# leggedrobotics/art_planner

Hardware: AMD Instinct MI355X
Metric: validated states/sec on 400x400@0.04m map (sample + validity check) (higher is better)
Workload: dtype f32; 1 GPU; C2: lazy_prm_star_min_update front end, 400x400@0.04m Perlin terrain (seed 1234) + 12 obstacles, YAML robot, batch sampler + validity checker; map=400x400@0.04, lanes=1

## Files before the change

### art_planner_amd/csrc/artp_capi.hip

```cpp
#include "../../include/artp_c.h"

#include <hip/hip_runtime.h>
#include <hipcub/hipcub.hpp>

#include <cmath>
#include <cstdio>
#include <atomic>
#include <chrono>
#include <cstdlib>
#include <cstring>
#include <mutex>
#include <string>
#include <array>
#include <vector>

#include "device_scratch.h"
#include "pinned_buffer.h"
#include "pipeline.h"
#include "cost_kernels.h"

using namespace artp;

#define ARTP_FEW_STATES 16
#define ARTP_SVC_MAX_STATES 2
// ... 1236 lines not shown
  if (exit_codes) HIP_TRY(c, hipMemcpyAsync(exit_codes, d_ec, n, hipMemcpyDeviceToHost, c->lane->stream));
  return check_error_flag(c);
}

int artp_validate_states_dev(artp_ctx* c, const double* se3, size_t n, uint8_t* valid, int8_t* detail) {
  if (!c || (n && (!se3 || !valid))) return ARTP_ERR_INVALID_ARG;
  std::lock_guard<std::recursive_mutex> lock(c->mu);
  if (!c->have_field[0] || !c->have_field[1]) return ARTP_ERR_NO_MAP;
  if (n == 0) return ARTP_OK;
  HIP_TRY(c, hipSetDevice(c->device));
  if (!detail && n <= ARTP_FEW_STATES) {
    hipLaunchKernelGGL(validate_few_kernel, dim3((unsigned)n), dim3(320), lds_few(c), c->lane->stream, c->field[0],
                       c->field[1], c->geom, c->robot, se3, n, valid, c->caps_full, c->caps_foot_full, c->lane->d_error.get(), 0u);
    HIP_TRY(c, hipGetLastError());
    return ARTP_OK;
  }
  if (detail) {
    hipLaunchKernelGGL(validate_states_kernel<1>, dim3(grid_full(c, n)), dim3(64), lds_full(c), c->lane->stream,
                       c->field[0], c->field[1], c->geom, c->robot, se3, n, valid, detail, c->caps_full,
                       c->lane->d_error.get(), (unsigned long long*)nullptr);
    HIP_TRY(c, hipGetLastError());
    return ARTP_OK;
  }
  return launch_validate_pipeline(c, se3, n, valid);
}

int artp_validate_states(artp_ctx* c, const double* se3, size_t n, uint8_t* valid, int8_t* detail) {
  if (!c || (n && (!se3 || !valid))) return ARTP_ERR_INVALID_ARG;
  if (n == 0) return ARTP_OK;
  std::lock_guard<std::recursive_mutex> lock(c->mu);
  HIP_TRY(c, hipSetDevice(c->device));
  if (!detail && n <= ARTP_FEW_STATES) {
    if (!c->have_field[0] || !c->have_field[1]) return ARTP_ERR_NO_MAP;
    if (c->svc_enabled && n <= ARTP_SVC_MAX_STATES) return svc_validate(c, se3, n, valid);
    std::memcpy(c->pin_states.host(), se3, n * 7 * sizeof(double));
    for (size_t i = 0; i < n; ++i) c->pin_labels.host()[i] = 0;
    const unsigned tag = 0x80u;
    hipLaunchKernelGGL(validate_few_kernel, dim3((unsigned)n), dim3(320), lds_few(c), c->lane->stream, c->field[0],
                       c->field[1], c->geom, c->robot, (const double*)c->pin_states.dev(), n,
                       (volatile uint8_t*)c->pin_labels.dev(), c->caps_full, c->caps_foot_full, c->lane->d_error.get(), tag);
    HIP_TRY(c, hipGetLastError());
    bool done = false;
    if (c->poll_labels) {
      const auto t0 = std::chrono::steady_clock::now();
      for (unsigned spin = 0; !done; ++spin) {
        done = true;
        for (size_t i = 0; i < n; ++i) done = done && (c->pin_labels.host()[i] & 0x80u);
        if (!done && (spin & 1023u) == 1023u &&
            std::chrono::steady_clock::now() - t0 > std::chrono::milliseconds(2))
          break;
      }
    }
    if (!done) HIP_TRY(c, hipStreamSynchronize(c->lane->stream));
    bool overflow = false;
    for (size_t i = 0; i < n; ++i) {
      valid[i] = c->pin_labels.host()[i] & 1u;
      overflow = overflow || (c->pin_labels.host()[i] & 2u);
    }
    if (overflow) {
      c->last_error = "a box window exceeded the LDS tile capacity";
      return ARTP_ERR_CAPACITY;
    }
    return ARTP_OK;
  }
  ARTP_TRY(ensure_scratch(c, c->lane->host_args, n * 7 * sizeof(double)));
  ARTP_TRY(ensure_scratch(c, c->lane->host_results, n * 7));
  HIP_TRY(c, hipMemcpyAsync(c->lane->host_args.get(), se3, n * 7 * sizeof(double), hipMemcpyHostToDevice, c->lane->stream));
  uint8_t* d_valid = c->lane->host_results.as<uint8_t>();
  int8_t* d_detail = reinterpret_cast<int8_t*>(d_valid + n);
  ARTP_TRY(artp_validate_states_dev(c, c->lane->host_args.as<const double>(), n, d_valid,
                                detail ? d_detail : nullptr));
  HIP_TRY(c, hipMemcpyAsync(valid, d_valid, n, hipMemcpyDeviceToHost, c->lane->stream));
  if (detail) HIP_TRY(c, hipMemcpyAsync(detail, d_detail, n * 6, hipMemcpyDeviceToHost, c->lane->stream));
  return check_error_flag(c);
}

static int pack_sampler_tables(artp_ctx* c, int rows, int cols);

static int ensure_sampler_storage(artp_ctx* c, int rows, int cols) {
  if (c->sampler_buf.get() && c->sampler_pack.get() && c->sampler_rows == rows && c->sampler_cols == cols) return ARTP_OK;
  const size_t e = (size_t)rows * cols;
  const int npiv = (cols + 15) / 16, pitch = npiv * 16, ppitch = (npiv + 3) & ~3;
  const size_t floats = (size_t)rows * pitch + (size_t)rows * ppitch + 8 * e + 64;
  for (lane_state& l : c->lanes)
    if (&l != c->lane && l.init) HIP_TRY(c, hipStreamSynchronize(l.stream));
  HIP_TRY(c, hipStreamSynchronize(c->lane->stream));
  c->have_sampler = false;
  c->sampler_rows = c->sampler_cols = 0;
  HIP_TRY(c, c->sampler_buf.reset());
  HIP_TRY(c, c->sampler_pack.reset());
  HIP_TRY(c, c->sampler_buf.reserve((6 * e + rows) * sizeof(float)));
  HIP_TRY(c, c->sampler_pack.reserve(floats * sizeof(float)));
  c->sampler_rows = rows;
  c->sampler_cols = cols;
  return ARTP_OK;
}

int artp_upload_sampler_layers(artp_ctx* c, const float* cum_prob, const float* cum_prob_rowwise,
                               const float* elevation, const float* normal_x, const float* normal_y,
                               const float* normal_z, const float* plane_fit_std_dev, int rows,
                               int cols, double len_x, double len_y, double pos_x, double pos_y) {
  if (!c || !cum_prob || !cum_prob_rowwise || !elevation || !normal_x || !normal_y || !normal_z ||
      !plane_fit_std_dev || rows < 1 || cols < 1)
    return ARTP_ERR_INVALID_ARG;
  std::lock_guard<std::recursive_mutex> lock(c->mu);
  HIP_TRY(c, hipSetDevice(c->device));
  const size_t e = (size_t)rows * cols;
  c->map_version.fetch_add(1, std::memory_order_release);
  ARTP_TRY(ensure_sampler_storage(c, rows, cols));
  ARTP_TRY(order_after_other_lanes(c));
  float* p = c->sampler_buf.get();
  const float* src[6] = {cum_prob, elevation, normal_x, normal_y, normal_z, plane_fit_std_dev};
  const float** dst[6] = {&c->sampler.cum_prob, &c->sampler.elevation, &c->sampler.normal_x,
                          &c->sampler.normal_y, &c->sampler.normal_z, &c->sampler.plane_fit_std_dev};
  for (int k = 0; k < 6; ++k) {
    HIP_TRY(c, hipMemcpyAsync(p, src[k], e * sizeof(float), hipMemcpyHostToDevice, c->lane->stream));
    *dst[k] = p;
    p += e;
  }
  HIP_TRY(c, hipMemcpyAsync(p, cum_prob_rowwise, rows * sizeof(float), hipMemcpyHostToDevice, c->lane->stream));
  c->sampler.cum_prob_rowwise = p;
  HIP_TRY(c, hipStreamSynchronize(c->lane->stream));
  ARTP_TRY(pack_sampler_tables(c, rows, cols));
  if (!c->have_geom) {
    c->geom.len_x = len_x; c->geom.len_y = len_y; c->geom.pos_x = pos_x; c->geom.pos_y = pos_y;
    c->geom.rows = rows; c->geom.cols = cols; c->geom.res = len_x / rows;
    c->have_geom = true;
  }
  c->sampler.from_distribution = c->params.sample_from_distribution;
  c->have_sampler = true;
  return publish_map_write(c);
}

static int pack_sampler_tables(artp_ctx* c, int rows, int cols) {
  const size_t e = (size_t)rows * cols;
  const int npiv = (cols + 15) / 16, pitch = npiv * 16, ppitch = (npiv + 3) & ~3;
  const size_t floats = (size_t)rows * pitch + (size_t)rows * ppitch + 8 * e + 64;
  HIP_TRY(c, hipMemsetAsync(c->sampler_pack.get(), 0, floats * sizeof(float), c->lane->stream));
  float* cells = c->sampler_pack.get();
  float* cdf_t = cells + 8 * e;
  float* piv = cdf_t + (size_t)rows * pitch;
  c->sampler.npiv = npiv;
  c->sampler.pitch = pitch;
  c->sampler.ppitch = ppitch;
  hipLaunchKernelGGL(sampler_pack_kernel, dim3((unsigned)((e + 255) / 256)), dim3(256), 0, c->lane->stream, c->sampler, rows,
                     cols, cdf_t, piv, reinterpret_cast<float4*>(cells));
  HIP_TRY(c, hipGetLastError());
  c->sampler.cells = reinterpret_cast<const float4*>(cells);
  c->sampler.cum_prob_t = cdf_t;
  c->sampler.pivots = piv;
  HIP_TRY(c, hipStreamSynchronize(c->lane->stream));
  return ARTP_OK;
}

static int upload_sampler_layers_from_device(artp_ctx* c, const float* cum_prob, const float* cum_prob_rowwise,
                                      const float* elevation, const float* normal_x, const float* normal_y,
                                      const float* normal_z, const float* plane_fit_std_dev, int rows, int cols,
                                      double len_x, double len_y, double pos_x, double pos_y) {
  std::lock_guard<std::recursive_mutex> lock(c->mu);
  HIP_TRY(c, hipSetDevice(c->device));
  const size_t e = (size_t)rows * cols;
  c->map_version.fetch_add(1, std::memory_order_release);
  ARTP_TRY(ensure_sampler_storage(c, rows, cols));
  ARTP_TRY(order_after_other_lanes(c));
  float* p = c->sampler_buf.get();
  const float* src[6] = {cum_prob, elevation, normal_x, normal_y, normal_z, plane_fit_std_dev};
  const float** dst[6] = {&c->sampler.cum_prob, &c->sampler.elevation, &c->sampler.normal_x,
                          &c->sampler.normal_y, &c->sampler.normal_z, &c->sampler.plane_fit_std_dev};
  for (int k = 0; k < 6; ++k) {
    HIP_TRY(c, hipMemcpyAsync(p, src[k], e * sizeof(float), hipMemcpyDeviceToDevice, c->lane->stream));
    *dst[k] = p;
    p += e;
  }
  HIP_TRY(c, hipMemcpyAsync(p, cum_prob_rowwise, rows * sizeof(float), hipMemcpyDeviceToDevice, c->lane->stream));
  c->sampler.cum_prob_rowwise = p;
  HIP_TRY(c, hipStreamSynchronize(c->lane->stream));
  ARTP_TRY(pack_sampler_tables(c, rows, cols));
  if (!c->have_geom) {
    c->geom.len_x = len_x; c->geom.len_y = len_y; c->geom.pos_x = pos_x; c->geom.pos_y = pos_y;
    c->geom.rows = rows; c->geom.cols = cols; c->geom.res = len_x / rows;
    c->have_geom = true;
  }
  c->sampler.from_distribution = c->params.sample_from_distribution;
  c->have_sampler = true;
  return publish_map_write(c);
}

static int finite_min_max_dev(artp_ctx* c, const float* d_layer, size_t n, float* lo, float* hi, bool* any) {
  std::lock_guard<std::recursive_mutex> lock(c->mu);
  HIP_TRY(c, hipSetDevice(c->device));
  int init[2] = {0x7fffffff, (int)0x80000000};
  int* d_keys = reinterpret_cast<int*>(c->lane->d_count.get());
  HIP_TRY(c, hipMemcpyAsync(d_keys, init, sizeof(init), hipMemcpyHostToDevice, c->lane->stream));
  hipLaunchKernelGGL(finite_min_max_kernel, dim3((unsigned)std::min<size_t>((n + 255) / 256, (size_t)c->n_cus)), dim3(256), 0,
                     c->lane->stream, d_layer, (int)n, d_keys);
  HIP_TRY(c, hipGetLastError());
  int keys[2];
  HIP_TRY(c, hipMemcpyAsync(keys, d_keys, sizeof(keys), hipMemcpyDeviceToHost, c->lane->stream));
  HIP_TRY(c, hipStreamSynchronize(c->lane->stream));
  *any = keys[0] <= keys[1];
  auto unkey = [](int k) {
    const int i = k >= 0 ? k : k ^ 0x7fffffff;
    float v;
    std::memcpy(&v, &i, 4);
    return v;
  };
  *lo = unkey(keys[0]);
  *hi = unkey(keys[1]);
  return ARTP_OK;
}

static int launch_sampler(artp_ctx* c, uint64_t seed, uint64_t first_index, size_t n, double* se3_out, PoseRec* recs) {
  const size_t blocks = (n + 255) / 256;
  if (blocks > 0x7fffffffull) {
    c->last_error = "batch too large for one sampler launch";
    return ARTP_ERR_INVALID_ARG;
  }
  if (c->sampler.from_distribution)
    hipLaunchKernelGGL(sample_states_kernel<true>, dim3((unsigned)blocks), dim3(256), 0, c->lane->stream, c->sampler,
                       c->geom, c->robot, seed, first_index, n, se3_out, c->field[0], recs);
  else
    hipLaunchKernelGGL(sample_states_kernel<false>, dim3((unsigned)blocks), dim3(256), 0, c->lane->stream, c->sampler,
                       c->geom, c->robot, seed, first_index, n, se3_out, c->field[0], recs);
  HIP_TRY(c, hipGetLastError());
  return ARTP_OK;
}

int artp_sample_states_dev(artp_ctx* c, uint64_t seed, uint64_t first_index, size_t n, double* se3_out) {
  if (!c || (n && !se3_out)) return ARTP_ERR_INVALID_ARG;
  std::lock_guard<std::recursive_mutex> lock(c->mu);
  if (!c->have_sampler) return ARTP_ERR_NO_MAP;
  if (n == 0) return ARTP_OK;
  HIP_TRY(c, hipSetDevice(c->device));
  return launch_sampler(c, seed, first_index, n, se3_out, nullptr);
}

int artp_sample_states(artp_ctx* c, uint64_t seed, uint64_t first_index, size_t n, double* se3_out) {
  if (!c || (n && !se3_out)) return ARTP_ERR_INVALID_ARG;
  if (n == 0) return ARTP_OK;
  std::lock_guard<std::recursive_mutex> lock(c->mu);
  HIP_TRY(c, hipSetDevice(c->device));
  ARTP_TRY(ensure_scratch(c, c->lane->host_args, n * 7 * sizeof(double)));
  ARTP_TRY(artp_sample_states_dev(c, seed, first_index, n, c->lane->host_args.as<double>()));
  HIP_TRY(c, hipMemcpyAsync(se3_out, c->lane->host_args.get(), n * 7 * sizeof(double), hipMemcpyDeviceToHost, c->lane->stream));
  HIP_TRY(c, hipStreamSynchronize(c->lane->stream));
  return ARTP_OK;
}

int artp_sample_and_validate_dev(artp_ctx* c, uint64_t seed, uint64_t first_index, size_t n,
                                 double* se3_out, uint8_t* valid_out, size_t* n_valid) {
  if (!c || (n && (!se3_out || !valid_out))) return ARTP_ERR_INVALID_ARG;
  std::lock_guard<std::recursive_mutex> lock(c->mu);
  if (!c->have_sampler || !c->have_field[0] || !c->have_field[1]) return ARTP_ERR_NO_MAP;
  if (n == 0) {
    if (n_valid) *n_valid = 0;
    return ARTP_OK;
  }
  if (n >= (1ull << 32)) {
    c->last_error = "batch too large (state index is 32 bit)";
    return ARTP_ERR_INVALID_ARG;
  }
  HIP_TRY(c, hipSetDevice(c->device));
  ARTP_TRY(ensure_recs(c, n));
  if (n <= ARTP_FEW_STATES) {
    ARTP_TRY(launch_sampler(c, seed, first_index, n, se3_out, nullptr));
    ARTP_TRY(artp_validate_states_dev(c, se3_out, n, valid_out, nullptr));
  } else {
    ARTP_TRY(launch_sampler(c, seed, first_index, n, se3_out, c->lane->pose_recs.as<PoseRec>()));
  }
  if (n > ARTP_FEW_STATES) {
    ARTP_TRY(launch_validate_pipeline(c, se3_out, n, valid_out, true));
  }
  if (n_valid) {
    HIP_TRY(c, hipMemsetAsync(c->lane->d_count.get(), 0, sizeof(unsigned long long), c->lane->stream));
    size_t blocks = (n / 16 + 255) / 256 + 1;
    if (blocks > (size_t)c->n_cus * 4) blocks = (size_t)c->n_cus * 4;
    hipLaunchKernelGGL(count_valid_kernel, dim3((unsigned)blocks), dim3(256), 0, c->lane->stream,
                       (const uint8_t*)valid_out, n, c->lane->d_count.get());
    HIP_TRY(c, hipGetLastError());
  }
  if (n_valid) {
    unsigned long long cnt = 0;
    HIP_TRY(c, hipMemcpyAsync(&cnt, c->lane->d_count.get(), sizeof(cnt), hipMemcpyDeviceToHost, c->lane->stream));
    HIP_TRY(c, hipStreamSynchronize(c->lane->stream));
    *n_valid = (size_t)cnt;
  }
  return ARTP_OK;
}

int artp_sample_and_validate(artp_ctx* c, uint64_t seed, uint64_t first_index, size_t n, double* se3_out,
                             uint8_t* valid_out, uint64_t* map_version) {
  if (!c || (n && (!se3_out || !valid_out))) return ARTP_ERR_INVALID_ARG;
  std::lock_guard<std::recursive_mutex> lock(c->mu);
  if (map_version) *map_version = c->map_version.load(std::memory_order_acquire);
  if (n == 0) return ARTP_OK;
  HIP_TRY(c, hipSetDevice(c->device));
  ARTP_TRY(ensure_scratch(c, c->lane->host_args, n * 7 * sizeof(double)));
  ARTP_TRY(ensure_scratch(c, c->lane->host_results, n));
  ARTP_TRY(artp_sample_and_validate_dev(c, seed, first_index, n, c->lane->host_args.as<double>(),
                                    c->lane->host_results.as<uint8_t>(), nullptr));
  HIP_TRY(c, hipMemcpyAsync(se3_out, c->lane->host_args.get(), n * 7 * sizeof(double), hipMemcpyDeviceToHost, c->lane->stream));
  HIP_TRY(c, hipMemcpyAsync(valid_out, c->lane->host_results.get(), n, hipMemcpyDeviceToHost, c->lane->stream));
  return check_error_flag(c);
}

int artp_set_r3_extent(artp_ctx* c, double max_extent) {
// ... 1701 lines not shown
```

### art_planner_amd/csrc/artp_math.h

```cpp
#pragma once

#include <hip/hip_runtime.h>
#include <stdint.h>

#define ARTP_HD __host__ __device__ __forceinline__
#define ARTP_EPS 1.1920928955078125e-07f

namespace artp {

struct FieldDev {
  const float* data;
  int nW, nD;
  float width, depth, half_w, half_d;
  float sample_w, sample_d, inv_w, inv_d, zx_aspect;
  float pos[3];
  float R[12];
  int has_nan;
  float partner_tol;
  const unsigned char* partner_flags;
  int partner_R;
};

template <class T>
ARTP_HD T gather32(const T* __restrict__ base, unsigned idx) {
  return *reinterpret_cast<const T*>(reinterpret_cast<const char*>(base) + idx * (unsigned)sizeof(T));
}

struct BoxHF {
  float pos[3];
  float R[9];
  float side[3];
  float aabb[6];
  int minX, maxX, minZ, maxZ;
  int on_field;
};

ARTP_HD float dot3(float a0, float a1, float a2, float b0, float b1, float b2) {
  return a0 * b0 + a1 * b1 + a2 * b2;
}

ARTP_HD bool is_finite(float v) { return (__float_as_uint(v) & 0x7f800000u) != 0x7f800000u; }
ARTP_HD bool is_nan(float v) { return v != v; }

ARTP_HD float next_toward_neg_inf(float x) {
  uint32_t u = __float_as_uint(x);
  if ((u & 0x7f800000u) == 0x7f800000u) return x;
  if ((u << 1) == 0u) return __uint_as_float(0x80000001u);
  return __uint_as_float((u & 0x80000000u) ? u + 1u : u - 1u);
}
ARTP_HD float next_toward_pos_inf(float x) {
  uint32_t u = __float_as_uint(x);
  if ((u & 0x7f800000u) == 0x7f800000u) return x;
  if ((u << 1) == 0u) return __uint_as_float(0x00000001u);
  return __uint_as_float((u & 0x80000000u) ? u - 1u : u + 1u);
}

ARTP_HD void safe_normalize3(float& a0, float& a1, float& a2) {
  const float abs0 = fabsf(a0), abs1 = fabsf(a1), abs2 = fabsf(a2);
  int idx;
  if (abs1 > abs0) {
    idx = (abs2 > abs1) ? 2 : 1;
  } else if (abs2 > abs0) {
    idx = 2;
  } else {
    if (!(abs0 > 0.0f)) return;
    idx = 0;
  }
  const float big = idx == 0 ? a0 : (idx == 1 ? a1 : a2);
  const float first = idx == 0 ? a1 : a0;
  const float second = idx == 2 ? a1 : a2;
  const float recip = 1.0f / fabsf(big);
  const float p1 = first * recip, p2 = second * recip;
  const float l = 1.0f / sqrtf(1.0f + p1 * p1 + p2 * p2);
  const float nb = copysignf(l, big), n1 = p1 * l, n2 = p2 * l;
  a0 = idx == 0 ? nb : n1;
  a1 = idx == 1 ? nb : (idx == 0 ? n1 : n2);
  a2 = idx == 2 ? nb : n2;
}

ARTP_HD void orthogonalize_R9(float& m0, float& m1, float& m2, float& m4, float& m5, float& m6, float& m8,
                              float& m9, float& m10) {
  if (!(m0 != 0.0f || m1 != 0.0f || m2 != 0.0f)) return;
  const float n0 = m0 * m0 + m1 * m1 + m2 * m2;
  const float proj = dot3(m0, m1, m2, m4, m5, m6);
  float r0 = m4, r1 = m5, r2 = m6;
  const bool in_place = !(proj != 0);
  if (!in_place) {
    const float pd = proj / n0;
    r0 = m4 - pd * m0;
    r1 = m5 - pd * m1;
    r2 = m6 - pd * m2;
  }
  if (!(r0 != 0.0f || r1 != 0.0f || r2 != 0.0f)) return;
  if (n0 != 1.0f) safe_normalize3(m0, m1, m2);
  const float n1 = r0 * r0 + r1 * r1 + r2 * r2;
  if (n1 != 1.0f) safe_normalize3(r0, r1, r2);
  if (in_place) {
    m4 = r0;
    m5 = r1;
    m6 = r2;
  }
  m8 = m1 * r2 - m2 * r1;
  m9 = m2 * r0 - m0 * r2;
  m10 = m0 * r1 - m1 * r0;
}

ARTP_HD void orthogonalize_R(float* m) {
  orthogonalize_R9(m[0], m[1], m[2], m[4], m[5], m[6], m[8], m[9], m[10]);
// ... 253 lines not shown
```

### art_planner_amd/csrc/kernels.h

```cpp
#pragma once

#include "box_check.h"

namespace artp {

struct RobotDev {
  float torso[3];
  float foot[3];
  float torso_off[3];
  float feet_off_x, feet_off_y;
  int unknown_space_untraversable;
  double reach_z;
  double max_pitch_pert, max_roll_pert;
};

struct MapGeom {
  double len_x, len_y, pos_x, pos_y, res;
  int rows, cols;
};

struct SamplerDev {
  int from_distribution;
  const float* cum_prob;
  const float* cum_prob_rowwise;
// ... 54 lines not shown
  return s;
}

__device__ __forceinline__ bool map_is_inside(const MapGeom& g, double px, double py) {
  const double tx = -((px - g.pos_x) - 0.5 * g.len_x);
  const double ty = -((py - g.pos_y) - 0.5 * g.len_y);
  return tx >= 0.0 && ty >= 0.0 && tx < g.len_x && ty < g.len_y;
}

template <int WAVES>
__global__ void __launch_bounds__(64 * WAVES)
check_boxes_kernel(FieldDev f, float sx, float sy, float sz, const float* __restrict__ poses,
                   size_t n, uint8_t* __restrict__ hit, uint8_t* __restrict__ exit_codes,
                   ScratchCaps caps, int* __restrict__ error_flag) {
  extern __shared__ __attribute__((aligned(16))) char smem[];
  const int lane = threadIdx.x & 63;
  const int wave_in_block = threadIdx.x >> 6;
  const WaveScratch s = carve_scratch(smem, wave_in_block, caps);
  const size_t wave0 = (size_t)blockIdx.x * WAVES + wave_in_block;
  const size_t stride = (size_t)gridDim.x * WAVES;
  for (size_t i = wave0; i < n; i += stride) {
    float pose[16];
#pragma unroll
    for (int k = 0; k < 16; ++k) pose[k] = poses[16 * i + k];
    BoxHF b;
    setup_box(f, pose, sx, sy, sz, b);
    int ec;
    const int r = wave_check_box(f, b, s, lane, &ec);
    if (r < 0) {
      if (lane == 0) atomicExch(error_flag, 1);
    }
    if (lane == 0) {
      hit[i] = (uint8_t)(r > 0);
      if (exit_codes) exit_codes[i] = (uint8_t)(ec < 0 ? 255 : ec);
    }
    wave_lds_sync();
  }
}

__device__ __forceinline__ void rot_from_quat(float x, float y, float z, float w, float R[9]) {
  const float tx = 2.0f * x, ty = 2.0f * y, tz = 2.0f * z;
  const float twx = tx * w, twy = ty * w, twz = tz * w;
  const float txx = tx * x, txy = ty * x, txz = tz * x;
  const float tyy = ty * y, tyz = tz * y, tzz = tz * z;
  R[0] = 1.0f - (tyy + tzz);
  R[1] = txy - twz;
  R[2] = txz + twy;
  R[3] = txy + twz;
  R[4] = 1.0f - (txx + tzz);
  R[5] = tyz - twx;
  R[6] = txz - twy;
  R[7] = tyz + twx;
  R[8] = 1.0f - (txx + tyy);
}

__device__ __forceinline__ void pose3_from_se3(const double* se3, float t[3], float R[9]) {
  t[0] = (float)se3[0];
  t[1] = (float)se3[1];
  t[2] = (float)se3[2];
  rot_from_quat((float)se3[3], (float)se3[4], (float)se3[5], (float)se3[6], R);
}

struct __attribute__((aligned(16))) PoseRec {
  float t[3];
  float q[4];
  float bR[9];
};

__device__ __forceinline__ void make_pose_rec(const FieldDev& f, const double* se3, float4 out[4]) {
  float t[3], R[9], bR[9];
  pose3_from_se3(se3, t, R);
  box_rotation_in_field(f, R, bR);
  out[0] = make_float4(t[0], t[1], t[2], (float)se3[3]);
  out[1] = make_float4((float)se3[4], (float)se3[5], (float)se3[6], bR[0]);
  out[2] = make_float4(bR[1], bR[2], bR[3], bR[4]);
  out[3] = make_float4(bR[5], bR[6], bR[7], bR[8]);
}

__device__ __forceinline__ int rec_stage_slot(int l, int k) { return 4 * l + ((k + (l >> 2)) & 3); }
__device__ __forceinline__ void stage_pose_rec(float4* rw, int lane, const float4 r[4]) {
#pragma unroll
  for (int k = 0; k < 4; ++k) rw[rec_stage_slot(lane, k)] = r[k];
}
__device__ __forceinline__ void flush_pose_recs(const float4* rw, int lane, size_t live, PoseRec* __restrict__ dst_recs) {
  float4* dst = reinterpret_cast<float4*>(dst_recs);
#pragma unroll
  for (int k = 0; k < 4; ++k) {
    const int j = k * 64 + lane;
    typedef float native_f4 __attribute__((ext_vector_type(4)));
    if ((size_t)j < live * 4)
      __builtin_nontemporal_store(reinterpret_cast<const native_f4*>(rw)[rec_stage_slot(j >> 2, j & 3)],
                                  reinterpret_cast<native_f4*>(dst) + j);
  }
}

__global__ void __launch_bounds__(256)
pose_rec_kernel(FieldDev f, const double* __restrict__ se3, size_t n, PoseRec* __restrict__ recs) {
  __shared__ double stage[4][64 * 8];
  const int lane = threadIdx.x & 63;
  double* sw = stage[threadIdx.x >> 6];
  const size_t i0 = (size_t)blockIdx.x * blockDim.x + (threadIdx.x - lane);
  if (i0 >= n) return;
  const size_t live = n - i0 < 64 ? n - i0 : 64;
  const double* in = se3 + 7 * i0;
  double v7[7];
#pragma unroll
  for (int k = 0; k < 7; ++k) v7[k] = in[(size_t)(k * 64 + lane) < live * 7 ? k * 64 + lane : 0];
#pragma unroll
  for (int k = 0; k < 7; ++k)
    if ((size_t)(k * 64 + lane) < live * 7) sw[k * 64 + lane] = v7[k];
  wave_lds_sync();
  float4 r[4];
  const bool have = (size_t)lane < live;
  if (have) {
    double st[7];
#pragma unroll
    for (int j = 0; j < 7; ++j) st[j] = sw[lane * 7 + j];
    make_pose_rec(f, st, r);
  }
  wave_lds_sync();
  float4* rw = reinterpret_cast<float4*>(sw);
  if (have) stage_pose_rec(rw, lane, r);
  wave_lds_sync();
  flush_pose_recs(rw, lane, live, recs + i0);
}

__device__ __forceinline__ int wave_state_valid(const FieldDev& fb, const FieldDev& ff,
                                                const MapGeom& g, const RobotDev& rb,
                                                const double* se3, const WaveScratch& s, int lane,
                                                int8_t* detail6) {
  float t[3], R[9];
  pose3_from_se3(se3, t, R);
  if (detail6 && lane == 0) {
#pragma unroll
    for (int k = 0; k < 5; ++k) detail6[k] = -2;
    detail6[5] = 0;
  }
  int valid = 1;
  int err = 0;
  for (int k = 0; k < 5 && valid; ++k) {
    const bool body = (k == 0);
    const float ox = body ? rb.torso_off[0] : ((k <= 2) ? rb.feet_off_x : -rb.feet_off_x);
    const float oy = body ? rb.torso_off[1] : ((k & 1) ? rb.feet_off_y : -rb.feet_off_y);
    const float oz = body ? rb.torso_off[2] : 0.0f;
    float pose[16];
    pose[0] = (R[0] * ox + (R[1] * oy + R[2] * oz)) + t[0];
    pose[1] = (R[3] * ox + (R[4] * oy + R[5] * oz)) + t[1];
    pose[2] = (R[6] * ox + (R[7] * oy + R[8] * oz)) + t[2];
    pose[3] = 0.0f;
#pragma unroll
    for (int r = 0; r < 3; ++r) {
      pose[4 + 4 * r + 0] = R[3 * r + 0];
      pose[4 + 4 * r + 1] = R[3 * r + 1];
      pose[4 + 4 * r + 2] = R[3 * r + 2];
      pose[4 + 4 * r + 3] = 0.0f;
    }
    const bool inside = map_is_inside(g, (double)pose[0], (double)pose[1]);
    int ok;
    int ec = -1;
    if (!inside) {
      ok = body ? 1 : !rb.unknown_space_untraversable;
    } else {
      const FieldDev& fk = body ? fb : ff;
      BoxHF b;
      setup_box(fk, pose, body ? rb.torso[0] : rb.foot[0], body ? rb.torso[1] : rb.foot[1],
                body ? rb.torso[2] : rb.foot[2], b);
      int r = wave_check_box(fk, b, s, lane, &ec);
      wave_lds_sync();
      if (r < 0) {
        err = 1;
        r = 0;
      }
      ok = body ? !r : r;
// ... 134 lines not shown
  unsigned long long t_idle = t_start;
  uint32_t served = 0;
  const volatile uint32_t* line = reinterpret_cast<const volatile uint32_t*>(mb);
  for (;;) {
    if (k == 0) {
      uint32_t leave = 0, w = 0, seq;
      for (;;) {
        if (lane < 16) w = line[lane];
        seq = (uint32_t)__builtin_amdgcn_readfirstlane((int)w);
        if (seq != last_seq) break;
        const uint32_t nq = (uint32_t)__builtin_amdgcn_readlane((int)w, 1);
        const unsigned long long now = wall_clock64();
        if ((nq & 0x100u) || now - t_idle > ARTP_SVC_IDLE_TICKS || now - t_start > ARTP_SVC_LIFE_TICKS) {
          leave = 1;
          break;
        }
        __builtin_amdgcn_s_sleep(4);
      }
      if (!leave && lane < 16) w = line[lane];
      if (lane < 16) s_line[lane] = w;
      if (!leave && ((uint32_t)__builtin_amdgcn_readlane((int)w, 1) & 0xffu) > 1u && lane < 14)
        s_line[16 + lane] = reinterpret_cast<const volatile uint32_t*>(mb->state1)[lane];
      if (lane == 0) s_exit = leave;
    }
    __syncthreads();
    if (s_exit) {
      if (threadIdx.x == 0) {
        mb->running = 0u;
        __threadfence_system();
      }
      return;
    }
    const uint32_t seq = s_line[0];
    uint32_t n = s_line[1] & 0xffu;
    n = n < 1u ? 1u : (n > 2u ? 2u : n);
    uint32_t bits = 0;
    for (uint32_t i = 0; i < n; ++i) {
      double st[7];
#pragma unroll
      for (int j = 0; j < 7; ++j) {
        const uint32_t lo = s_line[(i ? 16 : 2) + 2 * j], hi = s_line[(i ? 16 : 2) + 2 * j + 1];
        st[j] = __longlong_as_double((long long)(((unsigned long long)hi << 32) | lo));
      }
      const int ok = few_box_ok(fb, ff, g, rb, st, k, s, lane);
      wave_lds_sync();
      if (lane == 0) box_ok[k] = ok;
      __syncthreads();
      if (threadIdx.x == 0) {
        bool err = false, v = true;
#pragma unroll
        for (int q = 0; q < 5; ++q) {
          err = err || box_ok[q] < 0;
          v = v && box_ok[q] > 0;
        }
        bits |= ((v && !err ? 1u : 0u) | (err ? 2u : 0u)) << (2 * i);
      }
      __syncthreads();
    }
    if (threadIdx.x == 0) {
      mb->resp = (seq << 8) | bits;
      __threadfence_system();
      ++served;
      mb->served = served;
    }
    last_seq = seq;
    t_idle = wall_clock64();
    __syncthreads();
  }
}

ARTP_HD double uniform01(uint64_t seed, uint64_t index, unsigned k) {
  uint64_t x = seed + 0x9E3779B97F4A7C15ULL * (index * 8u + (uint64_t)k + 1u);
  x ^= x >> 30;
  x *= 0xBF58476D1CE4E5B9ULL;
  x ^= x >> 27;
  x *= 0x94D049BB133111EBULL;
  x ^= x >> 31;
  x += seed;
  x ^= x >> 30;
  x *= 0xBF58476D1CE4E5B9ULL;
  x ^= x >> 27;
  x *= 0x94D049BB133111EBULL;
  x ^= x >> 31;
  return (double)(x >> 11) * (1.0 / 9007199254740992.0);
}

__device__ __forceinline__ void sincos_half_angle(double x, double* sn, double* cs) {
  const double kf = rint(x * 6.36619772367581382433e-01);
  const int k = (int)kf;
  double r = fma(-kf, 1.57079632673412561417e+00, x);
  r = fma(-kf, 6.07710050650619224932e-11, r);
  const double z = r * r;
  const double ps = fma(z, fma(z, fma(z, fma(z, fma(z, 1.58969099521155010221e-10, -2.50507602534068634195e-08),
                                                 2.75573137070700676789e-06),
                                          -1.98412698298579493134e-04),
                                   8.33333333332248946124e-03),
                        -1.66666666666666324348e-01);
  const double pc = fma(z, fma(z, fma(z, fma(z, fma(z, -1.13596475577881948265e-11, 2.08757232129817482790e-09),
                                                 -2.75573143513906633035e-07),
                                          2.48015872894767294178e-05),
                                   -1.38888888888741095749e-03),
                        4.16666666666666019037e-02);
  const double s0 = fma(r * z, ps, r);
  const double c0 = fma(z * z, pc, fma(-0.5, z, 1.0));
  const bool swap = (k & 1) != 0;
  const double sa = swap ? c0 : s0, ca = swap ? s0 : c0;
  *sn = (k & 2) ? -sa : sa;
  *cs = ((k + 1) & 2) ? -ca : ca;
}

template <bool FROM_DIST>
__device__ __forceinline__ void sample_one(const SamplerDev& sm, const MapGeom& g, const RobotDev& rb,
                                           uint64_t seed, uint64_t index, double out[7], const float* row_cdf) {
  double px, py;
  int cell_row = 0, cell_col = 0;
  if (FROM_DIST) {
    const double samp_col = uniform01(seed, index, 0);
    const double samp_row = uniform01(seed, index, 1);
    int lo = 0, hi = g.rows - 1;
    while (lo < hi) {
      const int mid = (lo + hi) >> 1;
      if ((double)row_cdf[mid] > samp_row) hi = mid; else lo = mid + 1;
    }
    const int row = lo;
    const float* prow = sm.pivots + (size_t)row * sm.ppitch;
    const int nch = sm.ppitch >> 2;
    if (nch <= 8) {
      const float uf = __double2float_rd(samp_col);
      const float4* p4 = reinterpret_cast<const float4*>(prow);
      lo = 0;
#pragma unroll
      for (int h = 0; h < 2; ++h) {
        float4 pv[4];
#pragma unroll
        for (int k = 0; k < 4; ++k)
          if (4 * h + k < nch) pv[k] = p4[4 * h + k];
#pragma unroll
        for (int k = 0; k < 4; ++k)
          if (4 * h + k < nch)
            lo += (!(pv[k].x > uf) ? 1 : 0) + (!(pv[k].y > uf) ? 1 : 0) + (!(pv[k].z > uf) ? 1 : 0) +
                  (!(pv[k].w > uf) ? 1 : 0);
      }
    } else {
      lo = 0;
      hi = sm.npiv - 1;
      while (lo < hi) {
        const int mid = (lo + hi) >> 1;
        if ((double)prow[mid] > samp_col) hi = mid; else lo = mid + 1;
      }
    }
    const int c0 = lo << 4;
    const int c1 = (c0 + 15 < g.cols - 1) ? c0 + 15 : g.cols - 1;
    const float4* grp = reinterpret_cast<const float4*>(sm.cum_prob_t + (size_t)row * sm.pitch + c0);
    int below = 0;
    const float uf_col = __double2float_rd(samp_col);
#pragma unroll
    for (int q4 = 0; q4 < 4; ++q4) {
      const float4 v = grp[q4];
      below += (c0 + 4 * q4 + 0 <= c1 && !(v.x > uf_col)) ? 1 : 0;
      below += (c0 + 4 * q4 + 1 <= c1 && !(v.y > uf_col)) ? 1 : 0;
      below += (c0 + 4 * q4 + 2 <= c1 && !(v.z > uf_col)) ? 1 : 0;
      below += (c0 + 4 * q4 + 3 <= c1 && !(v.w > uf_col)) ? 1 : 0;
    }
    const int col = (c0 + below < c1) ? c0 + below : c1;
    cell_row = row;
    cell_col = col;
    px = (g.pos_x + (0.5 * g.len_x - 0.5 * g.res)) + g.res * (double)(-row);
    py = (g.pos_y + (0.5 * g.len_y - 0.5 * g.res)) + g.res * (double)(-col);
  } else {
    const double lx = g.pos_x - g.len_x, hx = g.pos_x + g.len_x;
    const double ly = g.pos_y - g.len_y, hy = g.pos_y + g.len_y;
    for (unsigned a = 0;; ++a) {
      px = (hx - lx) * uniform01(seed, index, 8 + 3 * a) + lx;
      py = (hy - ly) * uniform01(seed, index, 8 + 3 * a + 1) + ly;
      if (map_is_inside(g, px, py) || a >= 255) break;
    }
  }
  int ri, ci;
  if (FROM_DIST) {
    ri = cell_row;
    ci = cell_col;
  } else {
    ri = (int)(-(((px - 0.5 * g.len_x) - g.pos_x) / g.res));
    ci = (int)(-(((py - 0.5 * g.len_y) - g.pos_y) / g.res));
  }
  const size_t ind = (size_t)ri + (size_t)ci * g.rows;
  const float4 ca = sm.cells[2 * ind], cb = sm.cells[2 * ind + 1];
  double v0 = px, v1 = py, v2 = (double)ca.x;
  const double nwx = (double)ca.y;
  const double nwy = (double)ca.z;
  const double nwz = (double)ca.w;
  const float sd = cb.x;
  const float sd_min = (0.5f < sd) ? 0.5f : sd;
  const double u_pert = uniform01(seed, index, 2);
  const double pert = ((1.0 - (-1.0)) * u_pert + (-1.0)) * (double)sd_min * rb.reach_z;
  v0 += nwx * pert;
  v1 += nwy * pert;
  v2 += nwz * pert;
  out[0] = v0;
  out[1] = v1;
  out[2] = v2;
  const double pi = 3.14159265358979323846;
  double rpy0 = pi * (-2.0 * uniform01(seed, index, 3) + 1.0);
  double rpy1 = acos(1.0 - 2.0 * uniform01(seed, index, 4)) - pi / 2.0;
  const double rpy2 = pi * (-2.0 * uniform01(seed, index, 5) + 1.0);
  double sy2s, sy2c, qw, qz;
  sincos_half_angle(0.5 * rpy2, &sy2s, &sy2c);
  {
    qw = sy2c;
    qz = sy2s;
    const double cyaw = qw * qw - qz * qz, syaw = (qw + qw) * qz;
    const double nbx = cyaw * nwx + syaw * nwy;
    const double nby = cyaw * nwy - syaw * nwx;
    const double nbz = nwz;
    rpy0 = -atan2(nby, nbz) + rpy0 * (rb.max_roll_pert * (1.0 / 1.57079632679489661923));
    rpy1 = atan2(nbx, nbz) + rpy1 * (rb.max_pitch_pert * (1.0 / 0.78539816339744830962));
  }
  {
    double cr, cp, sr, sp;
    sincos_half_angle(rpy0 * 0.5, &sr, &cr);
    sincos_half_angle(rpy1 * 0.5, &sp, &cp);
    const double cy = sy2c, sy = sy2s;
    out[6] = cy * cp * cr + sy * sp * sr;
    out[3] = cy * cp * sr - sy * sp * cr;
    out[4] = sy * cp * sr + cy * sp * cr;
    out[5] = sy * cp * cr - cy * sp * sr;
  }
}

#define ARTP_ROW_CDF_LDS 2048
__device__ __forceinline__ const float* stage_row_cdf(const SamplerDev& sm, const MapGeom& g, float* lds) {
  if (!sm.from_distribution || g.rows > ARTP_ROW_CDF_LDS) return sm.cum_prob_rowwise;
  for (int i = threadIdx.x; i < g.rows; i += blockDim.x) lds[i] = sm.cum_prob_rowwise[i];
  __syncthreads();
  return lds;
}

#ifndef ARTP_SAMPLER_WAVES
#define ARTP_SAMPLER_WAVES 5
#endif
template <bool FROM_DIST>
__global__ void __launch_bounds__(256) __attribute__((amdgpu_waves_per_eu(ARTP_SAMPLER_WAVES, ARTP_SAMPLER_WAVES)))
sample_states_kernel(SamplerDev sm, MapGeom g, RobotDev rb, uint64_t seed, uint64_t first_index,
                     size_t n, double* __restrict__ se3_out, FieldDev f, PoseRec* __restrict__ recs) {
  __shared__ double stage[4][64 * 8];
  __shared__ float row_cdf_lds[ARTP_ROW_CDF_LDS];
  const float* row_cdf = stage_row_cdf(sm, g, row_cdf_lds);
  const int lane = threadIdx.x & 63;
  double* sw = stage[threadIdx.x >> 6];
  const size_t i0 = (size_t)blockIdx.x * blockDim.x + (threadIdx.x - lane);
  if (i0 >= n) return;
  const size_t i = i0 + lane;
  float4 r[4];
  if (i < n) {
    double st[7];
    sample_one<FROM_DIST>(sm, g, rb, seed, first_index + i, st, row_cdf);
#pragma unroll
    for (int k = 0; k < 7; ++k) sw[lane * 7 + k] = st[k];
    if (recs) make_pose_rec(f, st, r);
  }
  wave_lds_sync();
  const size_t live = n - i0 < 64 ? n - i0 : 64;
  const size_t cnt = live * 7;
  double* out = se3_out + 7 * i0;
#pragma unroll
  for (int k = 0; k < 7; ++k)
    if ((size_t)(k * 64 + lane) < cnt) __builtin_nontemporal_store(sw[k * 64 + lane], &out[k * 64 + lane]);
  if (recs) {
    wave_lds_sync();
    float4* rw = reinterpret_cast<float4*>(sw);
    if (i < n) stage_pose_rec(rw, lane, r);
    wave_lds_sync();
    flush_pose_recs(rw, lane, live, recs + i0);
  }
}

template <bool FROM_DIST>
__global__ void __launch_bounds__(256)
sample_states_at_kernel(SamplerDev sm, MapGeom g, RobotDev rb, uint64_t seed, uint64_t base_index,
                        const uint32_t* __restrict__ idx, const unsigned long long* __restrict__ count,
                        size_t cap, double* __restrict__ se3_out) {
  __shared__ float row_cdf_lds[ARTP_ROW_CDF_LDS];
  const float* row_cdf = stage_row_cdf(sm, g, row_cdf_lds);
  const size_t n = (size_t)(*count) < cap ? (size_t)(*count) : cap;
  for (size_t i = (size_t)blockIdx.x * blockDim.x + threadIdx.x; i < n;
       i += (size_t)gridDim.x * blockDim.x) {
    double st[7];
    sample_one<FROM_DIST>(sm, g, rb, seed, base_index + idx[i], st, row_cdf);
#pragma unroll
    for (int k = 0; k < 7; ++k) se3_out[7 * i + k] = st[k];
  }
}

constexpr int ARTP_BITS_TILE = 1024;
__device__ __forceinline__ unsigned long long masked_word(const unsigned long long* __restrict__ b, size_t w, size_t words,
                                                          size_t prefix_bits) {
  if (w >= words) return 0ull;
  unsigned long long v = b[w];
  const size_t lo = w * 64;
  if (lo + 64 > prefix_bits) v = lo >= prefix_bits ? 0ull : (v & (~0ull >> (64 - (prefix_bits - lo))));
  return v;
}

__global__ void __launch_bounds__(256)
bits_word_offsets_kernel(const unsigned long long* __restrict__ bits, size_t words_per_rank, size_t words, size_t prefix_bits,
                         unsigned* __restrict__ offsets , unsigned* __restrict__ tile_tot ,
                         unsigned long long* __restrict__ counts) {
  __shared__ unsigned wave_sum[4];
  const int r = blockIdx.y, t = threadIdx.x, lane = t & 63, wave = t >> 6;
  const unsigned long long* b = bits + (size_t)r * words_per_rank;
  const size_t w0 = (size_t)blockIdx.x * ARTP_BITS_TILE + (size_t)t * 4;
  unsigned c[4], run = 0;
#pragma unroll
  for (int i = 0; i < 4; ++i) {
    c[i] = run;
    run += (unsigned)__popcll(masked_word(b, w0 + i, words, prefix_bits));
  }
  unsigned incl = run;
#pragma unroll
  for (int d = 1; d < 64; d <<= 1) {
    const unsigned v = __shfl_up(incl, d, 64);
    if (lane >= d) incl += v;
  }
  if (lane == 63) wave_sum[wave] = incl;
  __syncthreads();
  unsigned base = 0;
#pragma unroll
  for (int k = 0; k < 4; ++k)
    if (k < wave) base += wave_sum[k];
  const unsigned excl = base + incl - run;
#pragma unroll
  for (int i = 0; i < 4; ++i)
    if (w0 + i < words) offsets[(size_t)r * words + w0 + i] = excl + c[i];
  if (t == 255) {
    const unsigned tot = base + incl;
    tile_tot[(size_t)r * gridDim.x + blockIdx.x] = tot;
    atomicAdd(&counts[r], (unsigned long long)tot);
  }
}

struct RankBases { unsigned long long base[16]; };

__device__ __forceinline__ int select_bit64(unsigned long long v, int k) {
  int pos = 0;
#pragma unroll
  for (int w = 32; w >= 1; w >>= 1) {
    const int cnt = __popcll(v & ((1ull << w) - 1ull));
    if (k >= cnt) {
      k -= cnt;
      v >>= w;
      pos += w;
    }
  }
  return pos;
// ... 737 lines not shown
```

Baseline: 4.410 billion states/s.

## Hand-roll sampler math: custom acos/atan2, bit-trick RNG, 32-bit indexing, recs template

Replaces the sampler's libm acos and atan2 with inline polynomial versions that keep constants in scalar registers. It builds uniform doubles by bit assembly, applies sincos signs with XOR, and compares against float CDFs directly instead of widening to double. Table addressing moves to 32-bit offsets, with a new 4 GB guard on table size, and the recs branch becomes a template parameter with a wave-uniform index. The aim is fewer f64 instructions and less address arithmetic in a compute-heavy kernel, at the risk of small numeric differences from the library functions.

```diff
diff --git a/art_planner_amd/csrc/artp_capi.hip b/art_planner_amd/csrc/artp_capi.hip
--- a/art_planner_amd/csrc/artp_capi.hip
+++ b/art_planner_amd/csrc/artp_capi.hip
@@ -1342,6 +1342,10 @@
   const size_t e = (size_t)rows * cols;
   const int npiv = (cols + 15) / 16, pitch = npiv * 16, ppitch = (npiv + 3) & ~3;
   const size_t floats = (size_t)rows * pitch + (size_t)rows * ppitch + 8 * e + 64;
+  if (floats * sizeof(float) > 0xffffffffull) {
+    c->last_error = "sampler tables of 4 GB or more (about 1.2e8 cells): map too large for the sampler";
+    return ARTP_ERR_INVALID_ARG;
+  }
   for (lane_state& l : c->lanes)
     if (&l != c->lane && l.init) HIP_TRY(c, hipStreamSynchronize(l.stream));
   HIP_TRY(c, hipStreamSynchronize(c->lane->stream));
@@ -1476,12 +1480,10 @@
     c->last_error = "batch too large for one sampler launch";
     return ARTP_ERR_INVALID_ARG;
   }
-  if (c->sampler.from_distribution)
-    hipLaunchKernelGGL(sample_states_kernel<true>, dim3((unsigned)blocks), dim3(256), 0, c->lane->stream, c->sampler,
-                       c->geom, c->robot, seed, first_index, n, se3_out, c->field[0], recs);
-  else
-    hipLaunchKernelGGL(sample_states_kernel<false>, dim3((unsigned)blocks), dim3(256), 0, c->lane->stream, c->sampler,
-                       c->geom, c->robot, seed, first_index, n, se3_out, c->field[0], recs);
+  auto kernel = c->sampler.from_distribution ? (recs ? sample_states_kernel<true, true> : sample_states_kernel<true, false>)
+                                             : (recs ? sample_states_kernel<false, true> : sample_states_kernel<false, false>);
+  hipLaunchKernelGGL(kernel, dim3((unsigned)blocks), dim3(256), 0, c->lane->stream, c->sampler, c->geom, c->robot, seed,
+                     first_index, n, se3_out, c->field[0], recs);
   HIP_TRY(c, hipGetLastError());
   return ARTP_OK;
 }
diff --git a/art_planner_amd/csrc/artp_math.h b/art_planner_amd/csrc/artp_math.h
--- a/art_planner_amd/csrc/artp_math.h
+++ b/art_planner_amd/csrc/artp_math.h
@@ -24,6 +24,11 @@
 template <class T>
 ARTP_HD T gather32(const T* __restrict__ base, unsigned idx) {
   return *reinterpret_cast<const T*>(reinterpret_cast<const char*>(base) + idx * (unsigned)sizeof(T));
+}
+
+template <class T>
+ARTP_HD const T* at32(const T* __restrict__ base, unsigned idx) {
+  return reinterpret_cast<const T*>(reinterpret_cast<const char*>(base) + idx * (unsigned)sizeof(T));
 }
 
 struct BoxHF {
diff --git a/art_planner_amd/csrc/kernels.h b/art_planner_amd/csrc/kernels.h
--- a/art_planner_amd/csrc/kernels.h
+++ b/art_planner_amd/csrc/kernels.h
@@ -160,13 +160,14 @@
 #pragma unroll
   for (int k = 0; k < 4; ++k) rw[rec_stage_slot(lane, k)] = r[k];
 }
-__device__ __forceinline__ void flush_pose_recs(const float4* rw, int lane, size_t live, PoseRec* __restrict__ dst_recs) {
+template <class N>
+__device__ __forceinline__ void flush_pose_recs(const float4* rw, int lane, N live, PoseRec* __restrict__ dst_recs) {
   float4* dst = reinterpret_cast<float4*>(dst_recs);
 #pragma unroll
   for (int k = 0; k < 4; ++k) {
     const int j = k * 64 + lane;
     typedef float native_f4 __attribute__((ext_vector_type(4)));
-    if ((size_t)j < live * 4)
+    if ((N)j < live * 4)
       __builtin_nontemporal_store(reinterpret_cast<const native_f4*>(rw)[rec_stage_slot(j >> 2, j & 3)],
                                   reinterpret_cast<native_f4*>(dst) + j);
   }
@@ -467,9 +468,46 @@
   x ^= x >> 27;
   x *= 0x94D049BB133111EBULL;
   x ^= x >> 31;
+#if defined(__HIP_DEVICE_COMPILE__)
+  const uint32_t xl = (uint32_t)x, xh = (uint32_t)(x >> 32);
+  const int nb = (int)(xl << 20) >> 31;
+  const double d = __hiloint2double((int)((xh >> 12) | 0x3FF00000u), (int)((xh << 20) | (xl >> 12)));
+  const double c = __hiloint2double(0x3FF00000 + nb, nb);
+  return d - c;
+#else
   return (double)(x >> 11) * (1.0 / 9007199254740992.0);
-}
-
+#endif
+}
+
+__device__ __forceinline__ float uniform01_floor_float(double u) {
+  return (float)__hiloint2double(__double2hiint(u), (int)((unsigned)__double2loint(u) & 0xE0000000u));
+}
+
+#define ARTP_F64_BITS(u) __builtin_bit_cast(double, (unsigned long long)(u##ULL))
+
+__device__ __forceinline__ double fma_const(double a, double b, double c) {
+  double d;
+  asm("v_fma_f64 %0, %1, %2, %3" : "=v"(d) : "v"(a), "v"(b), "s"(c));
+  return d;
+}
+
+__device__ __forceinline__ double mul_in_order(double a, double b) {
+  double d;
+  asm("v_mul_f64 %0, %1, %2" : "=v"(d) : "v"(a), "v"(b));
+  return d;
+}
+__device__ __forceinline__ double add_in_order(double a, double b) {
+  double d;
+  asm("v_add_f64 %0, %1, %2" : "=v"(d) : "v"(a), "v"(b));
+  return d;
+}
+__device__ __forceinline__ double sub_in_order(double a, double b) {
+  double d;
+  asm("v_add_f64 %0, %1, -%2" : "=v"(d) : "v"(a), "v"(b));
+  return d;
+}
+
+template <bool SIGN_BITS = false>
 __device__ __forceinline__ void sincos_half_angle(double x, double* sn, double* cs) {
   const double kf = rint(x * 6.36619772367581382433e-01);
   const int k = (int)kf;
@@ -490,8 +528,91 @@
   const double c0 = fma(z * z, pc, fma(-0.5, z, 1.0));
   const bool swap = (k & 1) != 0;
   const double sa = swap ? c0 : s0, ca = swap ? s0 : c0;
-  *sn = (k & 2) ? -sa : sa;
-  *cs = ((k + 1) & 2) ? -ca : ca;
+  if (SIGN_BITS) {
+    const unsigned ks = (unsigned)k << 30, kc = ((unsigned)k + 1u) << 30;
+    *sn = __hiloint2double(__double2hiint(sa) ^ (int)(ks & 0x80000000u), __double2loint(sa));
+    *cs = __hiloint2double(__double2hiint(ca) ^ (int)(kc & 0x80000000u), __double2loint(ca));
+  } else {
+    *sn = (k & 2) ? -sa : sa;
+    *cs = ((k + 1) & 2) ? -ca : ca;
+  }
+}
+
+__device__ __forceinline__ double acos_unit(double x) {
+  const double ax = fabs(x);
+  const bool big = ax >= 0.5;
+  const double h = fma(ax, -0.5, 0.5);
+  const double r = big ? h : x * x;
+  double p = fma(r, ARTP_F64_BITS(0x3FA059859FEA6A70), ARTP_F64_BITS(0xBF90A5A378A05EAF));
+  p = fma_const(r, p, ARTP_F64_BITS(0x3F94052137024D6A));
+  p = fma_const(r, p, ARTP_F64_BITS(0x3F7AB3A098A70509));
+  p = fma_const(r, p, ARTP_F64_BITS(0x3F88ED60A300C8D2));
+  p = fma_const(r, p, ARTP_F64_BITS(0x3F8C6FA84B77012B));
+  p = fma_const(r, p, ARTP_F64_BITS(0x3F91C6C111DCCB70));
+  p = fma_const(r, p, ARTP_F64_BITS(0x3F96E89F0A0ADACF));
+  p = fma_const(r, p, ARTP_F64_BITS(0x3F9F1C72C668963F));
+  p = fma_const(r, p, ARTP_F64_BITS(0x3FA6DB6DB41CE4BD));
+  p = fma_const(r, p, ARTP_F64_BITS(0x3FB333333336FD5B));
+  p = fma_const(r, p, ARTP_F64_BITS(0x3FC5555555555380));
+  p = r * p;
+  if (!big) return fma(ARTP_F64_BITS(0x3FEDD9AD336A0500), ARTP_F64_BITS(0x3FFAF154EEB562D6), -fma(x, p, x));
+  const double y0 = __builtin_amdgcn_rsq(h);
+  const double g0 = h * y0, h0 = y0 * 0.5;
+  const double e0 = fma(-h0, g0, 0.5);
+  const double h1 = fma(h0, e0, h0), g1 = fma(g0, e0, g0);
+  const double s = fma(fma(-g1, g1, h), h1, g1);
+  const double s2 = s * s;
+  const double s2e = fma(s, s, -s2);
+  const double d0 = h - s2;
+  const double num = d0 + (((h - d0) - s2) - s2e);
+  const double den = s * 2.0;
+  const double q0 = __builtin_amdgcn_rcp(den);
+  const double q1 = fma(fma(-den, q0, 1.0), q0, q0);
+  const double q2 = fma(fma(-den, q1, 1.0), q1, q1);
+  const double c0 = num * q2;
+  const double c = fma(fma(-den, c0, num), q2, c0);
+  const double sh = s + c;
+  const double sl = c - (sh - s);
+  const double neg = fma(ARTP_F64_BITS(0x3FFDD9AD336A0500), ARTP_F64_BITS(0x3FFAF154EEB562D6), fma(sh, p, sh) * -2.0);
+  const double pos = (sh + fma(sh, p, sl)) * 2.0;
+  const double v = x < 0.0 ? neg : pos;
+  return x == 1.0 ? 0.0 : v;
+}
+
+__device__ __forceinline__ double atan2_lib(double y, double x) {
+  const double ay = fabs(y), ax = fabs(x);
+  const double q = __builtin_fmin(ax, ay) / __builtin_fmax(ax, ay);
+  const double t = q * q;
+  double p = fma(t, ARTP_F64_BITS(0x3EEBA404B5E68A13), ARTP_F64_BITS(0xBF23E260BD3237F4));
+  p = fma_const(t, p, ARTP_F64_BITS(0x3F4B2BB069EFB384));
+  p = fma_const(t, p, ARTP_F64_BITS(0xBF67952DAF56DE9B));
+  p = fma_const(t, p, ARTP_F64_BITS(0x3F7D6D43A595C56F));
+  p = fma_const(t, p, ARTP_F64_BITS(0xBF8C6EA4A57D9582));
+  p = fma_const(t, p, ARTP_F64_BITS(0x3F967E295F08B19F));
+  p = fma_const(t, p, ARTP_F64_BITS(0xBF9E9AE6FC27006A));
+  p = fma_const(t, p, ARTP_F64_BITS(0x3FA2C15B5711927A));
+  p = fma_const(t, p, ARTP_F64_BITS(0xBFA59976E82D3FF0));
+  p = fma_const(t, p, ARTP_F64_BITS(0x3FA82D5D6EF28734));
+  p = fma_const(t, p, ARTP_F64_BITS(0xBFAAE5CE6A214619));
+  p = fma_const(t, p, ARTP_F64_BITS(0x3FAE1BB48427B883));
+  p = fma_const(t, p, ARTP_F64_BITS(0xBFB110E48B207F05));
+  p = fma_const(t, p, ARTP_F64_BITS(0x3FB3B13657B87036));
+  p = fma_const(t, p, ARTP_F64_BITS(0xBFB745D119378E4F));
+  p = fma_const(t, p, ARTP_F64_BITS(0x3FBC71C717E1913C));
+  p = fma_const(t, p, ARTP_F64_BITS(0xBFC2492492376B7D));
+  p = fma_const(t, p, ARTP_F64_BITS(0x3FC99999999952CC));
+  p = fma_const(t, p, ARTP_F64_BITS(0xBFD5555555555523));
+  const double a = fma(q, t * p, q);
+  const bool xneg = __double2hiint(x) < 0;
+  const double pi = ARTP_F64_BITS(0x400921FB54442D18);
+  double v = ax < ay ? ARTP_F64_BITS(0x3FF921FB54442D18) - a : a;
+  v = xneg ? pi - v : v;
+  v = y == 0.0 ? (xneg ? pi : 0.0) : v;
+  const double diag = __builtin_copysign(xneg ? ARTP_F64_BITS(0x4002D97C7F3321D2) : ARTP_F64_BITS(0x3FE921FB54442D18), y);
+  const double inf = ARTP_F64_BITS(0x7FF0000000000000);
+  v = (ay == inf && ax == inf) ? diag : v;
+  v = __builtin_isunordered(x, y) ? ARTP_F64_BITS(0x7FF8000000000000) : v;
+  return __builtin_copysign(v, y);
 }
 
 template <bool FROM_DIST>
@@ -502,17 +623,18 @@
   if (FROM_DIST) {
     const double samp_col = uniform01(seed, index, 0);
     const double samp_row = uniform01(seed, index, 1);
+    const float uf_row = uniform01_floor_float(samp_row);
     int lo = 0, hi = g.rows - 1;
     while (lo < hi) {
       const int mid = (lo + hi) >> 1;
-      if ((double)row_cdf[mid] > samp_row) hi = mid; else lo = mid + 1;
+      if (row_cdf[mid] > uf_row) hi = mid; else lo = mid + 1;
     }
     const int row = lo;
-    const float* prow = sm.pivots + (size_t)row * sm.ppitch;
+    const unsigned prow = (unsigned)row * (unsigned)sm.ppitch;
     const int nch = sm.ppitch >> 2;
+    const float uf = uniform01_floor_float(samp_col);
     if (nch <= 8) {
-      const float uf = __double2float_rd(samp_col);
-      const float4* p4 = reinterpret_cast<const float4*>(prow);
+      const float4* p4 = reinterpret_cast<const float4*>(at32(sm.pivots, prow));
       lo = 0;
 #pragma unroll
       for (int h = 0; h < 2; ++h) {
@@ -531,21 +653,20 @@
       hi = sm.npiv - 1;
       while (lo < hi) {
         const int mid = (lo + hi) >> 1;
-        if ((double)prow[mid] > samp_col) hi = mid; else lo = mid + 1;
+        if (gather32(sm.pivots, prow + (unsigned)mid) > uf) hi = mid; else lo = mid + 1;
       }
     }
     const int c0 = lo << 4;
     const int c1 = (c0 + 15 < g.cols - 1) ? c0 + 15 : g.cols - 1;
-    const float4* grp = reinterpret_cast<const float4*>(sm.cum_prob_t + (size_t)row * sm.pitch + c0);
+    const float4* grp = reinterpret_cast<const float4*>(at32(sm.cum_prob_t, (unsigned)row * (unsigned)sm.pitch + (unsigned)c0));
     int below = 0;
-    const float uf_col = __double2float_rd(samp_col);
 #pragma unroll
     for (int q4 = 0; q4 < 4; ++q4) {
       const float4 v = grp[q4];
-      below += (c0 + 4 * q4 + 0 <= c1 && !(v.x > uf_col)) ? 1 : 0;
-      below += (c0 + 4 * q4 + 1 <= c1 && !(v.y > uf_col)) ? 1 : 0;
-      below += (c0 + 4 * q4 + 2 <= c1 && !(v.z > uf_col)) ? 1 : 0;
-      below += (c0 + 4 * q4 + 3 <= c1 && !(v.w > uf_col)) ? 1 : 0;
+      below += (c0 + 4 * q4 + 0 <= c1 && !(v.x > uf)) ? 1 : 0;
+      below += (c0 + 4 * q4 + 1 <= c1 && !(v.y > uf)) ? 1 : 0;
+      below += (c0 + 4 * q4 + 2 <= c1 && !(v.z > uf)) ? 1 : 0;
+      below += (c0 + 4 * q4 + 3 <= c1 && !(v.w > uf)) ? 1 : 0;
     }
     const int col = (c0 + below < c1) ? c0 + below : c1;
     cell_row = row;
@@ -569,8 +690,8 @@
     ri = (int)(-(((px - 0.5 * g.len_x) - g.pos_x) / g.res));
     ci = (int)(-(((py - 0.5 * g.len_y) - g.pos_y) / g.res));
   }
-  const size_t ind = (size_t)ri + (size_t)ci * g.rows;
-  const float4 ca = sm.cells[2 * ind], cb = sm.cells[2 * ind + 1];
+  const float4* cell = at32(sm.cells, 2u * ((unsigned)ri + (unsigned)ci * (unsigned)g.rows));
+  const float4 ca = cell[0], cb = cell[1];
   double v0 = px, v1 = py, v2 = (double)ca.x;
   const double nwx = (double)ca.y;
   const double nwy = (double)ca.z;
@@ -587,10 +708,10 @@
   out[2] = v2;
   const double pi = 3.14159265358979323846;
   double rpy0 = pi * (-2.0 * uniform01(seed, index, 3) + 1.0);
-  double rpy1 = acos(1.0 - 2.0 * uniform01(seed, index, 4)) - pi / 2.0;
+  double rpy1 = acos_unit(1.0 - 2.0 * uniform01(seed, index, 4)) - pi / 2.0;
   const double rpy2 = pi * (-2.0 * uniform01(seed, index, 5) + 1.0);
   double sy2s, sy2c, qw, qz;
-  sincos_half_angle(0.5 * rpy2, &sy2s, &sy2c);
+  sincos_half_angle<true>(0.5 * rpy2, &sy2s, &sy2c);
   {
     qw = sy2c;
     qz = sy2s;
@@ -598,25 +719,26 @@
     const double nbx = cyaw * nwx + syaw * nwy;
     const double nby = cyaw * nwy - syaw * nwx;
     const double nbz = nwz;
-    rpy0 = -atan2(nby, nbz) + rpy0 * (rb.max_roll_pert * (1.0 / 1.57079632679489661923));
-    rpy1 = atan2(nbx, nbz) + rpy1 * (rb.max_pitch_pert * (1.0 / 0.78539816339744830962));
+    rpy0 = -atan2_lib(nby, nbz) + rpy0 * (rb.max_roll_pert * (1.0 / 1.57079632679489661923));
+    rpy1 = atan2_lib(nbx, nbz) + rpy1 * (rb.max_pitch_pert * (1.0 / 0.78539816339744830962));
   }
   {
     double cr, cp, sr, sp;
-    sincos_half_angle(rpy0 * 0.5, &sr, &cr);
-    sincos_half_angle(rpy1 * 0.5, &sp, &cp);
+    sincos_half_angle<true>(rpy0 * 0.5, &sr, &cr);
+    sincos_half_angle<true>(rpy1 * 0.5, &sp, &cp);
     const double cy = sy2c, sy = sy2s;
-    out[6] = cy * cp * cr + sy * sp * sr;
-    out[3] = cy * cp * sr - sy * sp * cr;
-    out[4] = sy * cp * sr + cy * sp * cr;
-    out[5] = sy * cp * cr - cy * sp * sr;
+    const double ycc = cy * cp, yss = sy * sp, ysc = sy * cp, ycs = cy * sp;
+    out[6] = add_in_order(mul_in_order(cr, ycc), mul_in_order(sr, yss));
+    out[3] = sub_in_order(mul_in_order(sr, ycc), mul_in_order(cr, yss));
+    out[4] = add_in_order(mul_in_order(sr, ysc), mul_in_order(cr, ycs));
+    out[5] = sub_in_order(mul_in_order(cr, ysc), mul_in_order(sr, ycs));
   }
 }
 
 #define ARTP_ROW_CDF_LDS 2048
 __device__ __forceinline__ const float* stage_row_cdf(const SamplerDev& sm, const MapGeom& g, float* lds) {
   if (!sm.from_distribution || g.rows > ARTP_ROW_CDF_LDS) return sm.cum_prob_rowwise;
-  for (int i = threadIdx.x; i < g.rows; i += blockDim.x) lds[i] = sm.cum_prob_rowwise[i];
+  for (unsigned i = threadIdx.x; i < (unsigned)g.rows; i += blockDim.x) lds[i] = gather32(sm.cum_prob_rowwise, i);
   __syncthreads();
   return lds;
 }
@@ -624,7 +746,7 @@
 #ifndef ARTP_SAMPLER_WAVES
 #define ARTP_SAMPLER_WAVES 5
 #endif
-template <bool FROM_DIST>
+template <bool FROM_DIST, bool WITH_RECS>
 __global__ void __launch_bounds__(256) __attribute__((amdgpu_waves_per_eu(ARTP_SAMPLER_WAVES, ARTP_SAMPLER_WAVES)))
 sample_states_kernel(SamplerDev sm, MapGeom g, RobotDev rb, uint64_t seed, uint64_t first_index,
                      size_t n, double* __restrict__ se3_out, FieldDev f, PoseRec* __restrict__ recs) {
@@ -632,29 +754,29 @@
   __shared__ float row_cdf_lds[ARTP_ROW_CDF_LDS];
   const float* row_cdf = stage_row_cdf(sm, g, row_cdf_lds);
   const int lane = threadIdx.x & 63;
-  double* sw = stage[threadIdx.x >> 6];
-  const size_t i0 = (size_t)blockIdx.x * blockDim.x + (threadIdx.x - lane);
+  const int wave = __builtin_amdgcn_readfirstlane((int)(threadIdx.x >> 6));
+  double* sw = stage[wave];
+  const size_t i0 = (size_t)blockIdx.x * blockDim.x + (size_t)wave * 64;
   if (i0 >= n) return;
-  const size_t i = i0 + lane;
+  const unsigned live = n - i0 < 64 ? (unsigned)(n - i0) : 64u;
   float4 r[4];
-  if (i < n) {
+  if ((unsigned)lane < live) {
     double st[7];
-    sample_one<FROM_DIST>(sm, g, rb, seed, first_index + i, st, row_cdf);
+    sample_one<FROM_DIST>(sm, g, rb, seed, first_index + i0 + (unsigned)lane, st, row_cdf);
 #pragma unroll
     for (int k = 0; k < 7; ++k) sw[lane * 7 + k] = st[k];
-    if (recs) make_pose_rec(f, st, r);
+    if (WITH_RECS) make_pose_rec(f, st, r);
   }
   wave_lds_sync();
-  const size_t live = n - i0 < 64 ? n - i0 : 64;
-  const size_t cnt = live * 7;
+  const unsigned cnt = live * 7;
   double* out = se3_out + 7 * i0;
 #pragma unroll
   for (int k = 0; k < 7; ++k)
-    if ((size_t)(k * 64 + lane) < cnt) __builtin_nontemporal_store(sw[k * 64 + lane], &out[k * 64 + lane]);
-  if (recs) {
+    if ((unsigned)(k * 64 + lane) < cnt) __builtin_nontemporal_store(sw[k * 64 + lane], &out[(unsigned)(k * 64 + lane)]);
+  if (WITH_RECS) {
     wave_lds_sync();
     float4* rw = reinterpret_cast<float4*>(sw);
-    if (i < n) stage_pose_rec(rw, lane, r);
+    if ((unsigned)lane < live) stage_pose_rec(rw, lane, r);
     wave_lds_sync();
     flush_pose_recs(rw, lane, live, recs + i0);
   }
```

Result: no change. 4.404 billion states/s, median of 2 (-0.1%).
